# BBCG/epialleleR

Measured on AMD Instinct MI355X. Metric: Mreads/s generateCytosineReport (150 bp PE), higher is better.
Workload: dtype u8

## Files before the change

### epialleler_amd/csrc/cx_report.hip

```cpp
#include "common.hpp"
#include "tile_common.hpp"
#include <stdio.h>
#include <stdlib.h>
#include <string.h>

namespace epi {

#ifndef EPI_CX_WG
#define EPI_CX_WG 512
#endif
#ifndef EPI_CX_T1
#define EPI_CX_T1 2048
#endif
constexpr int CX_WG = EPI_CX_WG;
constexpr int CX_T1 = EPI_CX_T1;
constexpr int CX_CH = 16;
constexpr int CX_FLUSH_ROWS = 255;
constexpr int CX_SLAB_COV = 12;

struct __attribute__((packed, aligned(1))) U4u { uint32_t x, y, z, w; };

#ifndef EPI_CX_ABLATE
#define EPI_CX_ABLATE 0
#endif

struct Cx2Args {
  RowCols c;
  int64_t xm_cap;
  const Tile *tiles;
  uint32_t fill4;
  ClassLut lut_r;
  ClassLut lut_rx, lut_sx;
  ClassLut lut_s;
  ThrParams thr;
  const uint32_t *thr_tab;
  uint32_t ctx_of_plane;
  int32_t *pass_out;
  uint32_t *pool_key, *pool_meth, *pool_unmeth;
  uint32_t pool_cap;
  uint32_t *cursor;
  uint32_t slot_rows, ovf_base;
  uint32_t *tile_nrow, *tile_base;
  int32_t *slab;
  int heavy_rows;
  int heavy_chunk;
  int heavy_first;
  uint32_t *heavy_count, *heavy_max;
  uint32_t *heavy_list;
  int32_t *heavy_slab;
  uint32_t *deep_count, *deep_list;
  const uint32_t *tile_list, *tile_list_count;
  uint32_t *dbg;
  int64_t nrows;
  const uint32_t *prev_off, *prev_nrow;
  uint32_t *mismatch;
  int32_t *out[6];
  int64_t out_cap;
};

template <int T, int NP, bool LEAN = false> struct Cx2Lds {
  static constexpr int Q = T / 4;
  static constexpr int N_NARROW = 2 * NP * Q;
  static constexpr int N_CORR = 2 * Q;
  static constexpr int N_WIDE = LEAN ? 16 : 2 * NP * T;
  static constexpr int N_COV = T;
  unsigned long long *narrow, *corr;
  uint32_t *wide, *cov;
  uint32_t tid;
};

__device__ __forceinline__ uint32_t cx2_lut(uint32_t w, const ClassLut &X, uint32_t low8) {
  const uint32_t sel = (w & 0x0F0F0F0Fu) | low8;
  return __builtin_amdgcn_perm(X.lo1, X.lo0, sel) ^ __builtin_amdgcn_perm(X.hi1, X.hi0, sel ^ 0x08080808u);
}

template <int G>
__device__ __forceinline__ uint32_t cx2_group_sum(uint32_t v) {
  v += (uint32_t)__builtin_amdgcn_update_dpp(0, (int)v, 0xB1, 0xF, 0xF, true);
  v += (uint32_t)__builtin_amdgcn_update_dpp(0, (int)v, 0x4E, 0xF, 0xF, true);
  if (G >= 8) v += (uint32_t)__builtin_amdgcn_update_dpp(0, (int)v, 0x141, 0xF, 0xF, true);
  if (G >= 16) v += (uint32_t)__builtin_amdgcn_update_dpp(0, (int)v, 0x140, 0xF, 0xF, true);
  if (G >= 32) v += __shfl_xor(v, 16, 64);
  if (G >= 64) v += __shfl_xor(v, 32, 64);
  return v;
}

__device__ __forceinline__ int cx2_threshold(uint32_t n_m, uint32_t n_u, uint32_t o_m, uint32_t o_u, const ThrParams &prm) {
  int res = 0;
  if (n_m != 0) {
    const unsigned n_all = n_m + n_u;
    if (!(n_all < prm.min_n_ctx)) {
      const double frac = (double)n_m / (double)n_all;
      if (!(frac < prm.min_ctx_meth_frac)) {
        res = 1;
        if (o_m > 0) {
          const unsigned o_all = o_m + o_u;
          const double ofrac = (double)o_m / (double)o_all;
          if (ofrac > prm.max_ooctx_meth_frac) res = 0;
        }
      }
    }
  }
  return res;
}

__device__ __forceinline__ int cx2_threshold_tab(uint32_t n_m, uint32_t n_u, uint32_t o_m, uint32_t o_u, const ThrParams &prm,
                                                 const uint32_t *__restrict__ tab) {
  const uint32_t n_all = n_m + n_u, o_all = o_m + o_u;
  const uint32_t least = tab[n_all] & 0xFFFFu, most = tab[o_all] >> 16;
  return n_m != 0u && !(n_all < prm.min_n_ctx) && n_m >= least && (o_m == 0u || o_m <= most);
}

__global__ __launch_bounds__(256) void k_thr_table(ThrParams prm, int32_t nmax, uint32_t *__restrict__ tab) {
  const int32_t n = (int32_t)(blockIdx.x * 256 + threadIdx.x);
  if (n > nmax) return;
  uint32_t least = 0xFFFFu, most = 0u;
  if (n >= 1) {
    int32_t lo = 1, hi = n + 1;
    while (lo < hi) {
      const int32_t m = (lo + hi) >> 1;
// ... 117 lines not shown
#pragma unroll
    for (int u = 0; u < NU; u++) {
#pragma unroll
      for (int d = 0; d < 4; d++) w[u][d] = (EPI_CX_ABLATE & 4) ? w[u][d] : cx2_lut(w[u][d], a.lut_sx, 0u);
      fl |= w[u][0] | w[u][1] | w[u][2] | w[u][3];
    }
    auto count = [&](auto masked) {
      constexpr bool MASKED = decltype(masked)::value;
      constexpr uint32_t EV = MASKED ? 0x55555555u : 0xFFFFFFFFu;
      uint32_t E = 0, O = 0;
#pragma unroll
      for (int u = 0; u < NU; u++) {
        const uint32_t t = (w[u][0] & EV) + (w[u][1] & EV) + (w[u][2] & EV);
        const uint32_t d3 = w[u][3] & EV;
        E += (t & 0x33333333u) + (d3 & 0x33333333u);
        O += ((t >> 2) & 0x33333333u) + ((d3 >> 2) & 0x33333333u);
        if (u % 3 == 2 || u == NU - 1) {
          cls[0] = __builtin_amdgcn_sad_u8(E & 0x0F0F0F0Fu, 0u, cls[0]);
          cls[2] = __builtin_amdgcn_sad_u8((E >> 4) & 0x0F0F0F0Fu, 0u, cls[2]);
          cls[1] = __builtin_amdgcn_sad_u8(O & 0x0F0F0F0Fu, 0u, cls[1]);
          cls[3] = __builtin_amdgcn_sad_u8((O >> 4) & 0x0F0F0F0Fu, 0u, cls[3]);
          E = 0; O = 0;
        }
      }
    };
    if constexpr (MODE != 2) {
      if (__builtin_expect(__ballot((fl & 0xAAAAAAAAu) != 0u) == 0ull, 1)) count(std::false_type{});
      else count(std::true_type{});
    }
    if constexpr (MODE == 1) {
#pragma unroll
      for (int k = 0; k < 4; k++) carry[k] += cls[k];
      return;
    }
    if constexpr (MODE == 0) {
      const uint32_t s01 = cx2_group_sum<G>(cls[0] | (cls[1] << 16)), s23 = cx2_group_sum<G>(cls[2] | (cls[3] << 16));
      const uint32_t n_all = s01 & 0xFFFFu, n_m = s01 >> 16;
      g.ps = a.thr_tab ? cx2_threshold_tab(n_m, n_all - n_m, s23 & 0xFFFFu, s23 >> 16, a.thr, a.thr_tab)
                       : cx2_threshold(n_m, n_all - n_m, s23 & 0xFFFFu, s23 >> 16, a.thr);
      if (a.pass_out && sub == 0 && (uint32_t)g.rel < (uint32_t)T) a.pass_out[rcur] = g.ps;
    }
    const uint32_t pm = g.ps ? 0x01010101u : 0u;
#pragma unroll
    for (int u = 0; u < NU; u++) {
      const bool inside = (uint32_t)(cb + u * G) < (uint32_t)C;
#pragma unroll
      for (int d = 0; d < 4; d++) {
        const uint32_t lo = w[u][d] & 0x01010101u, hi = (w[u][d] >> 2) & pm;
        if (lo != 0u && inside && !(EPI_CX_ABLATE & 2)) atomicAdd(nar + 4 * u * G + d, (unsigned long long)lo | ((unsigned long long)hi << 32));
      }
    }
    const uint32_t fsel = g.ps ? 0x0A0A0A0Au : 0xA0A0A0A0u;
    if (__builtin_expect((fl & fsel) != 0u, 0)) {
      const int sh = g.ps ? 1 : 5;
#pragma unroll
      for (int u = 0; u < NU; u++) {
        const bool inside = (uint32_t)(cb + u * G) < (uint32_t)C;
#pragma unroll
        for (int d = 0; d < 4; d++) {
          const uint32_t sk = (w[u][d] >> sh) & 0x01010101u, db = (w[u][d] >> (sh + 2)) & 0x01010101u;
          if ((sk | db) != 0u && inside) atomicAdd(cor + 4 * u * G + d, (unsigned long long)sk | ((unsigned long long)db << 32));
        }
      }
    }
  } else if constexpr (NP == 1 && G >= 16) {
    const bool passing = g.ps != 0;
    const uint32_t k77 = (a.ctx_of_plane & 255u) * 0x11111111u;
    const uint32_t rm = passing ? 0xDDDDDDDDu : 0x55555555u, rv = passing ? 0x99999999u : 0x11111111u;
    uint32_t clean = 0xFFFFFFFFu;
#pragma unroll
    for (int u = 0; u < NU; u++) {
      const bool inside = (uint32_t)(cb + u * G) < (uint32_t)C;
#pragma unroll
      for (int e = 0; e < 2; e++) {
        const uint32_t pk = (w[u][2 * e] & 0x0F0F0F0Fu) | ((w[u][2 * e + 1] << 4) & 0xF0F0F0F0u);
        const uint32_t z = ((pk & 0x77777777u) ^ k77) + 0x77777777u;
        const uint32_t np = ~z & 0x88888888u;
        const uint32_t t = (pk & rm) ^ rv;
        clean &= ((t & 0x77777777u) + 0x77777777u) | t;
        if (np != 0u && inside && !(EPI_CX_ABLATE & 2)) {
          const uint32_t up = passing ? np & ~pk : 0u;
          const uint32_t n0 = (np >> 3) & 0x01010101u, n1 = (np >> 7) & 0x01010101u;
          if (n0 != 0u) atomicAdd(nar + 4 * u * G + 2 * e, (unsigned long long)n0 | ((unsigned long long)((up >> 3) & 0x01010101u) << 32));
          if (n1 != 0u) atomicAdd(nar + 4 * u * G + 2 * e + 1, (unsigned long long)n1 | ((unsigned long long)((up >> 7) & 0x01010101u) << 32));
        }
      }
    }
    if (__builtin_expect((~clean & 0x88888888u) != 0u, 0)) {
      const uint32_t pick0 = passing ? 0u : 0x08080808u;
#pragma unroll
      for (int u = 0; u < NU; u++) {
        const bool inside = (uint32_t)(cb + u * G) < (uint32_t)C;
#pragma unroll
        for (int d = 0; d < 4; d++) {
          const uint32_t f = cx2_lut(w[u][d], a.lut_rx, pick0);
          const uint32_t sk = (f >> 6) & 0x01010101u, db = (f >> 7) & 0x01010101u;
          if ((sk | db) != 0u && inside) atomicAdd(cor + 4 * u * G + d, (unsigned long long)sk | ((unsigned long long)db << 32));
        }
      }
    }
  } else {
    const uint32_t pick0 = g.ps == 0 ? 0x08080808u : 0u;
    uint32_t fl = 0;
#pragma unroll
    for (int u = 0; u < NU; u++) {
      const bool inside = (uint32_t)(cb + u * G) < (uint32_t)C;
#pragma unroll
      for (int d = 0; d < 4; d++) {
        const uint32_t f = cx2_lut(w[u][d], a.lut_rx, pick0);
        w[u][d] = f;
        fl |= f;
#pragma unroll
        for (int p = 0; p < NP; p++) {
          const uint32_t lo = (f >> (2 * p)) & 0x01010101u, hi = (f >> (2 * p + 1)) & 0x01010101u;
          if (lo != 0u && inside && !(EPI_CX_ABLATE & 2))
            atomicAdd(nar + p * Q + 4 * u * G + d, (unsigned long long)lo | ((unsigned long long)hi << 32));
        }
      }
    }
    if (__builtin_expect((fl & 0xC0C0C0C0u) != 0u, 0)) {
#pragma unroll
      for (int u = 0; u < NU; u++) {
        const bool inside = (uint32_t)(cb + u * G) < (uint32_t)C;
#pragma unroll
        for (int d = 0; d < 4; d++) {
          const uint32_t sk = (w[u][d] >> 6) & 0x01010101u, db = (w[u][d] >> 7) & 0x01010101u;
          if ((sk | db) != 0u && inside) atomicAdd(cor + 4 * u * G + d, (unsigned long long)sk | ((unsigned long long)db << 32));
        }
      }
    }
  }
}

template <int T, int G, int NU, int NP, bool FUSED, int WG, class LT>
__device__ __forceinline__ void cx2_rows(const Cx2Args &a, const Tile &td, int row_lo, int row_hi, const LT &L) {
  constexpr int R = 64 / G, NW = WG / 64, C = T / CX_CH;
  const int lane = L.tid & 63, wave = L.tid >> 6;
  const int sub = lane & (G - 1), grp = lane / G;
  Tile tb = td;
  tb.row_hi = row_hi;
  int r = row_lo + wave * R + grp;
  RowVals v = cx_load_row(a.c, tb, r);
  for (int rbase = row_lo + wave * R; rbase < row_hi; rbase += NW * R) {
    const int rcur = r;
    if (!EPI_DEV_CHECK(a.dbg, !v.ok || (rcur >= 0 && rcur < a.nrows && v.len >= 0 && (v.sd == 1 || v.sd == 2 || v.len == 0)), 22, rcur, v.sd)) return;
    r += NW * R;
    RowVals nv;
    bool fetched = false;
    auto fetch_next = [&]() { if (!fetched) { nv = cx_load_row(a.c, tb, r); fetched = true; } };
    if (v.ok && v.len > 0 && (int32_t)((uint32_t)v.st - (uint32_t)td.pos0) + v.len > 0) {
      Cx2Row g;
      g.rel = (int32_t)((uint32_t)v.st - (uint32_t)td.pos0);
      g.len = v.len;
      g.c0 = g.rel >> 4;
      g.clast = (g.rel + v.len - 1) >> 4;
      g.base = a.c.xm + (v.o - g.rel);
      g.edge = v.o < CX_CH || v.o + v.len + CX_CH > a.xm_cap;
      g.sidx = v.sd - 1;
      g.ps = v.ps;
      if constexpr (FUSED) {
        if (__builtin_expect(__ballot(g.clast - g.c0 >= G * NU) == 0ull, 1)) {
          cx2_visit<T, G, NU, NP, true>(a, g, g.c0, g.clast, sub, rcur, L, fetch_next);
        } else {
          uint32_t cls[4] = {0, 0, 0, 0};
          for (int32_t cs = g.c0; __ballot(cs <= g.clast) != 0ull; cs += G * NU)
            cx2_visit<T, G, NU, NP, true, 1>(a, g, cs, g.clast, sub, rcur, L, fetch_next, cls);
          const uint32_t s01 = cx2_group_sum<G>(cls[0] | (cls[1] << 16)), s23 = cx2_group_sum<G>(cls[2] | (cls[3] << 16));
          const uint32_t n_all = s01 & 0xFFFFu, n_m = s01 >> 16;
          g.ps = a.thr_tab ? cx2_threshold_tab(n_m, n_all - n_m, s23 & 0xFFFFu, s23 >> 16, a.thr, a.thr_tab)
                           : cx2_threshold(n_m, n_all - n_m, s23 & 0xFFFFu, s23 >> 16, a.thr);
          if (a.pass_out && sub == 0 && (uint32_t)g.rel < (uint32_t)T) a.pass_out[rcur] = g.ps;
          const int32_t ca = g.c0 > 0 ? g.c0 : 0, cz = g.clast < C - 1 ? g.clast : C - 1;
          for (int32_t cs = ca; __ballot(cs <= cz) != 0ull; cs += G * NU)
// ... 7 lines not shown
          for (int32_t cs = ca; __ballot(cs <= cz) != 0ull; cs += G * NU) cx2_visit<T, G, NU, NP, false>(a, g, cs, cz, sub, rcur, L, fetch_next);
        }
      }
      if (sub == 0) {
        const int32_t ca = g.rel > 0 ? g.rel : 0, cb = g.rel + v.len < T ? g.rel + v.len : T;
        const uint32_t unit = g.sidx ? 65536u : 1u;
        if (ca < cb && !(EPI_CX_ABLATE & 32)) { atomicAdd(L.cov + ca, unit); if (cb < T) atomicAdd(L.cov + cb, 0u - unit); }
      }
    } else if (FUSED && v.ok && sub == 0 && a.pass_out && (uint32_t)((uint32_t)v.st - (uint32_t)td.pos0) < (uint32_t)T) {
      a.pass_out[rcur] = 0;
    }
    fetch_next();
    v = nv;
  }
}

template <int T, int NP, bool LEAN, int WG>
__device__ __forceinline__ void cx2_flush(const Cx2Lds<T, NP, LEAN> &L) {
  constexpr int Q = Cx2Lds<T, NP, LEAN>::Q;
  if constexpr (!LEAN) {
    for (int i = L.tid; i < 2 * NP * Q; i += WG) {
      const unsigned long long v = L.narrow[i];
      if (v == 0ull) continue;
      L.narrow[i] = 0ull;
      const uint32_t lo = (uint32_t)v, hi = (uint32_t)(v >> 32);
      const int sp = i / Q, q = i - sp * Q;
      uint4 *wd = reinterpret_cast<uint4 *>(L.wide + sp * T + 4 * q);
      uint4 c = *wd;
      c.x += (lo & 255u) | ((hi & 255u) << 16);
      c.y += ((lo >> 8) & 255u) | (((hi >> 8) & 255u) << 16);
      c.z += ((lo >> 16) & 255u) | (((hi >> 16) & 255u) << 16);
      c.w += (lo >> 24) | ((hi >> 24) << 16);
      *wd = c;
    }
  }
  for (int i = L.tid; i < 2 * Q; i += WG) {
    const unsigned long long v = L.corr[i];
    if (v == 0ull) continue;
    L.corr[i] = 0ull;
    const uint32_t sk = (uint32_t)v, db = (uint32_t)(v >> 32);
    const int s = i / Q, q = i - s * Q;
    const int32_t unit = s ? 65536 : 1;
    int32_t prev = 0;
#pragma unroll
    for (int j = 0; j < 4; j++) {
      const int32_t d = (int32_t)((db >> (8 * j)) & 255u) - (int32_t)((sk >> (8 * j)) & 255u);
      if (d != prev) atomicAdd(L.cov + 4 * q + j, (uint32_t)((d - prev) * unit));
      prev = d;
    }
    if (prev != 0 && 4 * q + 4 < T) atomicAdd(L.cov + 4 * q + 4, (uint32_t)(-prev * unit));
  }
}

__device__ __forceinline__ uint32_t cx_pool_reserve(const Cx2Args &a, int tile, uint32_t n, bool *fits) {
  if (n <= a.slot_rows) { *fits = true; return (uint32_t)tile * a.slot_rows; }
  const uint32_t o = atomicAdd(a.cursor, n);
  *fits = (uint64_t)a.ovf_base + o + n <= a.pool_cap;
  return a.ovf_base + o;
}

__device__ __forceinline__ void cx_direct_none(const Cx2Args &a, int tile, uint32_t tid = threadIdx.x) {
  if (a.prev_off && tid == 0 && a.prev_nrow[tile] != 0u) atomicAdd(a.mismatch, 1u);
}

template <int T, int NP> struct CxSrcLds {
  const uint32_t *wide, *cov;
  __device__ __forceinline__ uint32_t any(int sd, int pos) const {
    uint32_t x = 0;
#pragma unroll
    for (int p = 0; p < NP; p++) x |= wide[(sd * NP + p) * T + pos];
    return x;
  }
  __device__ __forceinline__ void pair(int sd, int p, int pos, uint32_t *n, uint32_t *M) const {
    const uint32_t w = wide[(sd * NP + p) * T + pos];
    *n = w & 0xFFFFu; *M = w >> 16;
  }
  __device__ __forceinline__ uint32_t coverage(int sd, int pos) const { const uint32_t v = cov[pos]; return sd ? v >> 16 : v & 0xFFFFu; }
};
template <int QS> struct CxSrcU8 {
  const uint32_t *narrow;
  const uint32_t *cov;
  __device__ __forceinline__ uint32_t any(int sd, int pos) const {
    return (narrow[2 * (sd * QS + (pos >> 2))] >> (8 * (pos & 3))) & 255u;
  }
  __device__ __forceinline__ void pair(int sd, int, int pos, uint32_t *n, uint32_t *M) const {
    const uint2 c = *reinterpret_cast<const uint2 *>(narrow + 2 * (sd * QS + (pos >> 2)));
    *n = (c.x >> (8 * (pos & 3))) & 255u; *M = (c.y >> (8 * (pos & 3))) & 255u;
  }
  __device__ __forceinline__ uint32_t coverage(int sd, int pos) const { const uint32_t v = cov[pos]; return sd ? v >> 16 : v & 0xFFFFu; }
};
template <int T, int NP> struct CxSrcSlab {
  const int32_t *slab;
  const uint32_t *cov;
  __device__ __forceinline__ uint32_t any(int sd, int pos) const {
    uint32_t x = 0;
#pragma unroll
    for (int p = 0; p < NP; p++) x |= (uint32_t)slab[(2 * (sd * NP + p)) * T + pos];
    return x;
  }
  __device__ __forceinline__ void pair(int sd, int p, int pos, uint32_t *n, uint32_t *M) const {
    *n = (uint32_t)slab[(2 * (sd * NP + p)) * T + pos]; *M = (uint32_t)slab[(2 * (sd * NP + p) + 1) * T + pos];
  }
  __device__ __forceinline__ uint32_t coverage(int sd, int pos) const { return cov[sd * T + pos]; }
};

template <int T, int WG = CX_WG>
__device__ __forceinline__ void cx2_prefix(uint32_t *arr, uint32_t *s_scan, uint32_t tid = threadIdx.x) {
  constexpr int PPT = T / WG, NW = WG / 64;
  static_assert(PPT >= 1 && PPT <= 8, "prefix layout");
  const int lane = tid & 63, wave = tid >> 6;
  uint32_t x[PPT];
#pragma unroll
  for (int j = 0; j < PPT; j++) x[j] = arr[tid * PPT + j];
#pragma unroll
  for (int j = 1; j < PPT; j++) x[j] += x[j - 1];
  const uint32_t inc = wave_scan_u32(x[PPT - 1]);
  if (lane == 63) s_scan[wave] = inc;
  __syncthreads();
  uint32_t before = inc - x[PPT - 1];
#pragma unroll
  for (int w = 0; w < NW; w++) before += w < wave ? s_scan[w] : 0u;
#pragma unroll
  for (int j = 0; j < PPT; j++) arr[tid * PPT + j] = x[j] + before;
  __syncthreads();
}

template <int T, int NP, int WG = CX_WG, class SRC>
__device__ __forceinline__ void cx2_emit(const Cx2Args &a, int tile, const SRC &src, uint32_t *s_scan, uint16_t *s_list, uint32_t tid = threadIdx.x) {
  constexpr int NW = WG / 64, PW = T / NW, IT = PW / 32;
  static_assert(PW % 32 == 0 && IT >= 1 && IT <= 16, "emit phase layout");
  const int lane = tid & 63, wave = tid >> 6;
  const int l5 = lane & 31, sd = lane >> 5;
  const uint32_t below = (1u << l5) - 1u;
  uint16_t *list = s_list + wave * (2 * PW);
  uint32_t nc = 0;
#pragma unroll
  for (int i = 0; i < IT; i++) {
    const uint32_t any = src.any(sd, wave * PW + i * 32 + l5);
    const unsigned long long bal = __ballot(any != 0u);
    const uint32_t blo = (uint32_t)bal, bhi = (uint32_t)(bal >> 32);
    const uint32_t rank = (uint32_t)__popc(blo & below) + (uint32_t)__popc(bhi & below) + (sd ? (blo >> l5) & 1u : 0u);
    if (any != 0u) list[nc + rank] = (uint16_t)(i * 64 + lane);
    nc += (uint32_t)__popcll(bal);
  }
  uint32_t key[IT], me[IT], un[IT], off[IT];
  bool ok[IT];
  uint32_t carry = 0;
#pragma unroll
  for (int jj = 0; jj < IT; jj++) {
    ok[jj] = false; key[jj] = 0; me[jj] = 0; un[jj] = 0; off[jj] = 0;
    if ((uint32_t)(jj * 64) < nc) {
      const uint32_t j = (uint32_t)(jj * 64 + lane);
      bool good = false;
      if (j < nc) {
        const uint32_t id = list[j];
        const int pos = wave * PW + (int)(id >> 6) * 32 + (int)(id & 31u), st = (int)((id >> 5) & 1u);
        const uint32_t half = src.coverage(st, pos) >> 1;
        uint32_t ctx = 0, m = 0, u = 0;
#pragma unroll
        for (int p = 0; p < NP; p++) {
          uint32_t nn, M;
          src.pair(st, p, pos, &nn, &M);
          if (nn > half && ctx == 0) { ctx = (a.ctx_of_plane >> (8 * p)) & 255u; m = M; u = nn - M; }
        }
        good = ctx != 0;
        key[jj] = ((uint32_t)pos << 4) | ((uint32_t)st << 3) | ctx;
        me[jj] = m;
        un[jj] = u;
      }
      const unsigned long long be = __ballot(good);
      off[jj] = carry + __builtin_amdgcn_mbcnt_hi((uint32_t)(be >> 32), __builtin_amdgcn_mbcnt_lo((uint32_t)be, 0u));
      carry += (uint32_t)__popcll(be);
      ok[jj] = good;
    }
  }
  if (lane == 0) s_scan[wave] = carry;
  __syncthreads();
  if (a.prev_off) {
    if (tid == 0) {
      uint32_t acc = 0;
      for (int w = 0; w < NW; w++) { const uint32_t t = s_scan[w]; s_scan[w] = acc; acc += t; }
      const uint32_t base = a.prev_off[tile];
      const bool good = acc == a.prev_nrow[tile] && (int64_t)base + acc <= a.out_cap;
      if (!good) atomicAdd(a.mismatch, 1u);
      s_scan[NW + 1] = good ? base : 0xFFFFFFFFu;
    }
    __syncthreads();
    const uint32_t base = s_scan[NW + 1];
    if (base != 0xFFFFFFFFu) {
      const Tile td = a.tiles[tile];
      const uint32_t w0 = base + s_scan[wave];
#pragma unroll
      for (int jj = 0; jj < IT; jj++) {
        if (ok[jj]) {
          const uint32_t o = w0 + off[jj];
          a.out[0][o] = td.rname;
          a.out[1][o] = 1 + (int32_t)((key[jj] >> 3) & 1u);
          a.out[2][o] = (int32_t)(td.pos0 + (int64_t)(key[jj] >> 4));
          a.out[3][o] = (int32_t)(key[jj] & 7u);
          a.out[4][o] = (int32_t)me[jj];
          a.out[5][o] = (int32_t)un[jj];
        }
      }
    }
    return;
  }
  if (tid == 0) {
    uint32_t acc = 0;
    for (int w = 0; w < NW; w++) { const uint32_t t = s_scan[w]; s_scan[w] = acc; acc += t; }
    s_scan[NW] = acc;
    uint32_t base = 0;
    bool fits = true;
    if (acc) base = cx_pool_reserve(a, tile, acc, &fits);
    s_scan[NW + 1] = base;
    s_scan[NW] = fits ? acc : 0xFFFFFFFFu;
    a.tile_nrow[tile] = acc;
    a.tile_base[tile] = base;
  }
  __syncthreads();
  const uint32_t total = s_scan[NW], base = s_scan[NW + 1];
  if (total != 0xFFFFFFFFu) {
    const uint32_t w0 = base + s_scan[wave];
#pragma unroll
    for (int jj = 0; jj < IT; jj++) {
      if (ok[jj]) {
        const uint32_t w = w0 + off[jj];
        if (!EPI_DEV_CHECK(a.dbg, w < a.pool_cap, 23, w, a.pool_cap)) continue;
        a.pool_key[w] = key[jj];
        a.pool_meth[w] = me[jj];
        a.pool_unmeth[w] = un[jj];
      }
    }
  }
}

template <int T, int NP, bool LEAN, int WG>
__device__ __forceinline__ void cx2_dump_slab(const Cx2Lds<T, NP, LEAN> &L, int32_t *slab) {
  uint32_t *dst = reinterpret_cast<uint32_t *>(slab);
  if constexpr (LEAN) {
    constexpr int Q = Cx2Lds<T, NP, LEAN>::Q;
    for (int i = L.tid; i < 2 * NP * Q; i += WG) {
      const unsigned long long v = L.narrow[i];
      if (v == 0ull) continue;
      const uint32_t lo = (uint32_t)v, hi = (uint32_t)(v >> 32);
      const int sp = i / Q, q = i - sp * Q;
#pragma unroll
      for (int j = 0; j < 4; j++) {
        const uint32_t n = (lo >> (8 * j)) & 255u, M = (hi >> (8 * j)) & 255u;
        if (n) atomicAdd(dst + (2 * sp) * T + 4 * q + j, n);
        if (M) atomicAdd(dst + (2 * sp + 1) * T + 4 * q + j, M);
      }
    }
  } else {
    for (int i = L.tid; i < 2 * NP * T; i += WG) {
      const uint32_t v = L.wide[i];
      if (!v) continue;
      const int sp = i / T, p = i - sp * T;
      if (v & 0xFFFFu) atomicAdd(dst + (2 * sp) * T + p, v & 0xFFFFu);
      if (v >> 16) atomicAdd(dst + (2 * sp + 1) * T + p, v >> 16);
    }
  }
  for (int p = L.tid; p < T; p += WG) {
    const uint32_t v = L.cov[p];
    if (!v) continue;
    const int32_t lo = (int32_t)(int16_t)(v & 0xFFFFu);
    const int32_t hi = ((int32_t)v - lo) >> 16;
    if (lo) atomicAdd(dst + CX_SLAB_COV * T + p, (uint32_t)lo);
    if (hi) atomicAdd(dst + (CX_SLAB_COV + 1) * T + p, (uint32_t)hi);
  }
}

__device__ __forceinline__ int cx_tile_of_block(int b, int ntiles) {
  const int chunk = (ntiles + 7) >> 3;
  return (b & 7) * chunk + (b >> 3);
}

template <int T, int NP, bool LEAN = false> constexpr int cx2_lds_bytes() {
  using LdsT = Cx2Lds<T, NP, LEAN>;
  return (LdsT::N_NARROW + LdsT::N_CORR) * 8 + (LdsT::N_WIDE + LdsT::N_COV) * 4;
}
#ifndef EPI_CX_WPS
#define EPI_CX_WPS 8
#endif
template <int T, int NP, int NU = 3, bool LEAN = false, int WG = CX_WG> constexpr int cx2_waves_per_simd() {
  const int by_lds = (160 * 1024) / (cx2_lds_bytes<T, NP, LEAN>() + 64), by_thr = 2048 / WG;
  int wgs = by_lds < by_thr ? by_lds : by_thr;
  if (NU >= 4 && wgs * WG > 1536) wgs = 1536 / WG;
  if (wgs * WG / 256 > EPI_CX_WPS) wgs = EPI_CX_WPS * 256 / WG;
  return (wgs < 1 ? 1 : wgs) * WG / 256;
}

#define CX2_SHARED(T, NP, LEAN)                                                                                  \
  using LdsT = Cx2Lds<T, NP, LEAN>;                                                                              \
  __shared__ __attribute__((aligned(16))) unsigned long long s_u8[LdsT::N_NARROW + LdsT::N_CORR];                \
  __shared__ __attribute__((aligned(16))) uint32_t s_wide[LdsT::N_WIDE];                                         \
  __shared__ __attribute__((aligned(16))) uint32_t s_cov[LdsT::N_COV];                                           \
  static_assert((LdsT::N_NARROW + LdsT::N_CORR) * 8 >= 4 * T + 64 && LdsT::N_CORR * 8 >= 4 * T, "the candidate lists and the scan scratch reuse dead arrays"); \
  uint32_t *s_scan = LEAN ? s_wide : reinterpret_cast<uint32_t *>(s_u8) + T;                                      \
  uint16_t *s_list = reinterpret_cast<uint16_t *>(LEAN ? s_u8 + LdsT::N_NARROW : s_u8);                          \
  (void)s_scan; (void)s_list;                                                                                     \
  LdsT L;                                                                                                         \
  L.narrow = s_u8; L.corr = s_u8 + LdsT::N_NARROW; L.wide = s_wide; L.cov = s_cov; L.tid = threadIdx.x;

template <int T, int NP, bool LEAN, int WG>
__device__ __forceinline__ void cx2_clear(const Cx2Lds<T, NP, LEAN> &L) {
  using LdsT = Cx2Lds<T, NP, LEAN>;
  uint4 *z = reinterpret_cast<uint4 *>(L.narrow);
  for (int i = L.tid; i < (LdsT::N_NARROW + LdsT::N_CORR) / 2; i += WG) z[i] = make_uint4(0, 0, 0, 0);
  if constexpr (!LEAN) {
    uint4 *y = reinterpret_cast<uint4 *>(L.wide);
    for (int i = L.tid; i < LdsT::N_WIDE / 4; i += WG) y[i] = make_uint4(0, 0, 0, 0);
  }
  uint4 *x = reinterpret_cast<uint4 *>(L.cov);
  for (int i = L.tid; i < LdsT::N_COV / 4; i += WG) x[i] = make_uint4(0, 0, 0, 0);
}

template <int T, int G, int NU, int NP, bool FUSED, bool LEAN, int WG>
__device__ __forceinline__ void cx2_accumulate(const Cx2Args &a, const Tile &td, int row_lo, int row_hi, const Cx2Lds<T, NP, LEAN> &L) {
  if constexpr (LEAN) {
    cx2_rows<T, G, NU, NP, FUSED, WG>(a, td, row_lo, row_hi, L);
  } else {
    for (int b0 = row_lo; b0 < row_hi; b0 += CX_FLUSH_ROWS) {
      if (b0 > row_lo) { __syncthreads(); cx2_flush<T, NP, LEAN, WG>(L); __syncthreads(); }
      cx2_rows<T, G, NU, NP, FUSED, WG>(a, td, b0, b0 + CX_FLUSH_ROWS < row_hi ? b0 + CX_FLUSH_ROWS : row_hi, L);
    }
  }
  __syncthreads();
  cx2_flush<T, NP, LEAN, WG>(L);
  __syncthreads();
}

#ifndef EPI_CX_LEAN_WG
#define EPI_CX_LEAN_WG 256
#endif
template <bool LEAN> constexpr int cx2_wg() { return LEAN ? EPI_CX_LEAN_WG : CX_WG; }

template <int T, int G, int NU, int NP, bool FUSED, bool LEAN, class LdsT>
__device__ __forceinline__ void cx2_tile(const Cx2Args &a, int tile, const Tile &td, const LdsT &L, uint32_t *s_scan, uint16_t *s_list, int *s_flag) {
  constexpr int WG = cx2_wg<LEAN>();
  cx2_clear<T, NP, LEAN, WG>(L);
  if (td.row_hi - td.row_lo > a.heavy_rows) {
    if (L.tid == 0) {
      const uint32_t h = atomicAdd(a.heavy_count, 1u);
      a.heavy_list[h] = (uint32_t)tile;
      atomicMax(a.heavy_max, (uint32_t)(td.row_hi - td.row_lo));
      a.tile_nrow[tile] = 0;
      a.tile_base[tile] = 0;
    }
    cx_direct_none(a, tile, L.tid);
    return;
  }
  if constexpr (LEAN) {
    if (a.deep_list && td.row_hi - td.row_lo > CX_FLUSH_ROWS) {
      if (L.tid == 0) *s_flag = 0;
      __syncthreads();
      bool deep = false;
      for (int x = td.row_lo + (int)L.tid; x + CX_FLUSH_ROWS < td.row_hi; x += WG)
        deep |= (int64_t)a.c.start[x + CX_FLUSH_ROWS] < (int64_t)a.c.start[x] + a.c.len[x];
      if (deep) *s_flag = 1;
      __syncthreads();
      if (*s_flag) {
        if (L.tid == 0) { a.deep_list[atomicAdd(a.deep_count, 1u)] = (uint32_t)tile; a.tile_nrow[tile] = 0; a.tile_base[tile] = 0; }
        cx_direct_none(a, tile, L.tid);
        return;
      }
    }
  }
  __syncthreads();
  cx2_accumulate<T, G, NU, NP, FUSED, LEAN, WG>(a, td, td.row_lo, td.row_hi, L);
  if (td.slot >= 0) {
    cx2_dump_slab<T, NP, LEAN, WG>(L, a.slab + (int64_t)td.slot * (kCxPlanes * T));
    if (L.tid == 0) { a.tile_nrow[tile] = 0; a.tile_base[tile] = 0; }
    cx_direct_none(a, tile, L.tid);
    return;
  }
  if (EPI_CX_ABLATE & 16) { if (L.tid == 0) { a.tile_nrow[tile] = 0; a.tile_base[tile] = 0; } cx_direct_none(a, tile, L.tid); return; }
  cx2_prefix<T, WG>(L.cov, s_scan, L.tid);
  if constexpr (LEAN) {
    static_assert(NP == 1, "the u8 counters serve single-context reports");
    CxSrcU8<LdsT::Q> src;
    src.narrow = reinterpret_cast<const uint32_t *>(L.narrow); src.cov = L.cov;
    cx2_emit<T, NP, WG>(a, tile, src, s_scan, s_list, L.tid);
  } else {
    CxSrcLds<T, NP> src;
    src.wide = L.wide; src.cov = L.cov;
    cx2_emit<T, NP, WG>(a, tile, src, s_scan, s_list, L.tid);
  }
}

template <int T, int G, int NU, int NP, bool FUSED, bool LEAN>
__global__ __launch_bounds__(cx2_wg<LEAN>(), (cx2_waves_per_simd<T, NP, NU, LEAN, cx2_wg<LEAN>()>())) void k_cx_tiles(Cx2Args a, int ntiles) {
  CX2_SHARED(T, NP, LEAN)
  __shared__ int s_flag;
  if constexpr (!LEAN) {
    if (a.tile_list) {
      const uint32_t n = *a.tile_list_count;
      for (uint32_t i = blockIdx.x; i < n; i += gridDim.x) {
        const int tile = (int)a.tile_list[i];
        const Tile td = a.tiles[tile];
        cx2_tile<T, G, NU, NP, FUSED, LEAN>(a, tile, td, L, s_scan, s_list, &s_flag);
        __syncthreads();
      }
      return;
    }
  }
  const int tile = cx_tile_of_block(blockIdx.x, ntiles);
  if (tile >= ntiles) return;
  const Tile td = a.tiles[tile];
  cx2_tile<T, G, NU, NP, FUSED, LEAN>(a, tile, td, L, s_scan, s_list, &s_flag);
}

template <int T, int G, int NU, int NP, bool FUSED>
__global__ __launch_bounds__(CX_WG, (cx2_waves_per_simd<T, NP, NU>())) void k_cx_heavy(Cx2Args a) {
  CX2_SHARED(T, NP, false)
  const uint32_t hi_idx = (uint32_t)a.heavy_first + blockIdx.y;
  if (hi_idx >= *a.heavy_count) return;
  const int tile = (int)a.heavy_list[hi_idx];
  const Tile td = a.tiles[tile];
  for (int lo = td.row_lo + (int)blockIdx.x * a.heavy_chunk; lo < td.row_hi; lo += (int)gridDim.x * a.heavy_chunk) {
    const int hi = td.row_hi - lo > a.heavy_chunk ? lo + a.heavy_chunk : td.row_hi;
    cx2_clear<T, NP, false, CX_WG>(L);
    __syncthreads();
    cx2_accumulate<T, G, NU, NP, FUSED, false, CX_WG>(a, td, lo, hi, L);
    cx2_dump_slab<T, NP, false, CX_WG>(L, td.slot >= 0 ? a.slab + (int64_t)td.slot * (kCxPlanes * T)
                                          : a.heavy_slab + (int64_t)blockIdx.y * (kCxPlanes * T));
    __syncthreads();
  }
}

template <int T, int NP>
__device__ __forceinline__ void cx2_emit_from_slab(const Cx2Args &a, int tile, const int32_t *slab) {
  __shared__ __attribute__((aligned(16))) uint32_t s_cov[2 * T];
  __shared__ uint32_t s_scan[CX_WG / 64 + 2];
  __shared__ uint16_t s_list[2 * T];
  for (int i = threadIdx.x; i < 2 * T; i += CX_WG) s_cov[i] = (uint32_t)slab[CX_SLAB_COV * T + i];
  __syncthreads();
  cx2_prefix<T>(s_cov, s_scan);
  cx2_prefix<T>(s_cov + T, s_scan);
  CxSrcSlab<T, NP> src;
  src.slab = slab; src.cov = s_cov;
  cx2_emit<T, NP>(a, tile, src, s_scan, s_list);
}

template <int T, int NP>
__global__ __launch_bounds__(CX_WG) void k_cx_emit_heavy(Cx2Args a) {
  const uint32_t hi_idx = (uint32_t)a.heavy_first + blockIdx.x;
  if (hi_idx >= *a.heavy_count) return;
  const int tile = (int)a.heavy_list[hi_idx];
  if (a.tiles[tile].slot >= 0) return;
  cx2_emit_from_slab<T, NP>(a, tile, a.heavy_slab + (int64_t)blockIdx.x * (kCxPlanes * T));
}

template <int T, int NP>
__global__ __launch_bounds__(CX_WG) void k_cx_emit_slab(Cx2Args a, const int32_t *__restrict__ owned,
                                                         const int32_t *__restrict__ slot_tile) {
  if (!owned[blockIdx.x]) return;
  const int tile = slot_tile[blockIdx.x];
  if (tile < 0) return;
  cx2_emit_from_slab<T, NP>(a, tile, a.slab + (int64_t)a.tiles[tile].slot * (kCxPlanes * T));
}

#ifndef EPI_CXP_T
#define EPI_CXP_T 1024
#endif
constexpr int CXP_T = EPI_CXP_T;

template <int G, int U0, int U1>
__device__ __forceinline__ void cxp_add_range(const uint32_t (&w)[CX_NU], const RowSlice &cur) {
  if constexpr (U0 < U1) {
    if (U0 * G <= cur.tl) cx_add_dword<CXP_T, 4 * G * U0, U0 == 0>(w[U0], cur.tl == U0 * G, cur);
    cxp_add_range<G, U0 + 1, U1>(w, cur);
  }
}

template <int G>
__device__ __forceinline__ void cxp_accumulate(const RowCols &c, const Tile &td, uint32_t *cnt) {
  constexpr int R = 64 / G, NW = CX_WG / 64;
  const int lane = threadIdx.x & 63, wave = threadIdx.x >> 6;
  const int sub = lane & (G - 1), grp = lane / G;
  int r = td.row_lo + wave * R + grp;
  RowSlice cur = cx_row_slice<CXP_T, G>(c, td, r, sub, cnt);
  for (int rbase = td.row_lo + wave * R; rbase < td.row_hi; rbase += NW * R) {
    uint32_t w[CX_NU];
#pragma unroll
    for (int u = 0; u < CX_NU; u++) w[u] = u * G <= cur.tl ? cur.src[u * G] : 0u;
    r += NW * R;
    const RowSlice nxt = cx_row_slice<CXP_T, G>(c, td, r, sub, cnt);
    cxp_add_range<G, 0, CX_NU>(w, cur);
    for (int k = sub + CX_NU * G; k < cur.nd; k += G) {
      RowSlice t = cur;
#pragma unroll
      for (int j = 0; j < 4; j++) t.dst[j] = cur.dst[j] + 4 * (k - sub);
      cx_add_dword<CXP_T, 0, false>(cur.src[k - sub], k == cur.nd - 1, t);
    }
// ... 18 lines not shown
  const uint32_t *cnt;
  int pl[3];
  __device__ __forceinline__ uint32_t any(int sd, int pos) const {
    uint32_t x = 0;
#pragma unroll
    for (int p = 0; p < 3; p++) if (pl[p]) x |= cnt[(sd * 4 + pl[p]) * CXP_T + pos];
    return x;
  }
  __device__ __forceinline__ void pair(int sd, int p, int pos, uint32_t *n, uint32_t *M) const {
    const uint32_t w = pl[p] ? cnt[(sd * 4 + pl[p]) * CXP_T + pos] : 0u;
    *n = w & 0xFFFFu; *M = w >> 16;
  }
  __device__ __forceinline__ uint32_t coverage(int sd, int pos) const { return cnt[sd * 4 * CXP_T + pos]; }
};

__device__ __forceinline__ CxSrcPk cxp_source(const Cx2Args &a, const uint32_t *cnt) {
  CxSrcPk s;
  s.cnt = cnt;
#pragma unroll
  for (int p = 0; p < 3; p++) { const uint32_t k = (a.ctx_of_plane >> (8 * p)) & 255u; s.pl[p] = k == 2u ? 1 : k == 6u ? 2 : k == 7u ? 3 : 0; }
  return s;
}

__device__ __forceinline__ void cxp_dump_slab(const Cx2Args &a, const uint32_t *cnt, int np, int32_t *slab) {
  constexpr int T = CXP_T;
  uint32_t *dst = reinterpret_cast<uint32_t *>(slab);
  const CxSrcPk src = cxp_source(a, cnt);
  for (int i = threadIdx.x; i < 2 * T; i += CX_WG) {
    const int sd = i / T, pos = i % T;
#pragma unroll
    for (int p = 0; p < 3; p++) {
      if (p >= np) break;
      uint32_t n, M;
      src.pair(sd, p, pos, &n, &M);
      if (n) atomicAdd(dst + (2 * (sd * np + p)) * T + pos, n);
      if (M) atomicAdd(dst + (2 * (sd * np + p) + 1) * T + pos, M);
    }
    const uint32_t d = src.coverage(sd, pos) - (pos ? src.coverage(sd, pos - 1) : 0u);
    if (d) atomicAdd(dst + (CX_SLAB_COV + sd) * T + pos, d);
  }
}

#define CXP_SHARED                                                                                      \
  __shared__ __attribute__((aligned(16))) uint32_t cnt_raw[8 * CXP_T + 2 * kCxGuard];                  \
  __shared__ uint32_t s_scan[CX_WG / 64 + 2];                                                         \
  __shared__ uint16_t s_list[2 * CXP_T];                                                               \
  uint32_t *cnt = cnt_raw + kCxGuard;

template <int G>
__global__ __launch_bounds__(CX_WG, 8) void k_cxp_tiles(Cx2Args a, int ntiles, int np) {
  CXP_SHARED
  const int tile = cx_tile_of_block(blockIdx.x, ntiles);
  if (tile >= ntiles) return;
  const Tile td = a.tiles[tile];
  uint4 *z = reinterpret_cast<uint4 *>(cnt_raw);
  for (int i = threadIdx.x; i < (8 * CXP_T + 2 * kCxGuard) / 4; i += CX_WG) z[i] = make_uint4(0, 0, 0, 0);
  if (td.row_hi - td.row_lo > a.heavy_rows) {
    if (threadIdx.x == 0) {
      const uint32_t h = atomicAdd(a.heavy_count, 1u);
      a.heavy_list[h] = (uint32_t)tile;
      atomicMax(a.heavy_max, (uint32_t)(td.row_hi - td.row_lo));
      a.tile_nrow[tile] = 0;
      a.tile_base[tile] = 0;
    }
    cx_direct_none(a, tile);
    return;
  }
  __syncthreads();
  cxp_accumulate<G>(a.c, td, cnt);
  __syncthreads();
  cxp_convert(cnt);
  __syncthreads();
  if (td.slot >= 0) {
    cxp_dump_slab(a, cnt, np, a.slab + (int64_t)td.slot * (kCxPlanes * CXP_T));
    if (threadIdx.x == 0) { a.tile_nrow[tile] = 0; a.tile_base[tile] = 0; }
    cx_direct_none(a, tile);
    return;
  }
  if (EPI_CX_ABLATE & 16) {
    if (threadIdx.x == 0) { a.tile_nrow[tile] = 0; a.tile_base[tile] = 0; }
    cx_direct_none(a, tile);
    return;
  }
  cx2_emit<CXP_T, 3>(a, tile, cxp_source(a, cnt), s_scan, s_list);
}

template <int G>
__global__ __launch_bounds__(CX_WG, 8) void k_cxp_heavy(Cx2Args a, int np) {
  CXP_SHARED
  (void)s_scan; (void)s_list;
  const uint32_t hi_idx = (uint32_t)a.heavy_first + blockIdx.y;
  if (hi_idx >= *a.heavy_count) return;
  const int tile = (int)a.heavy_list[hi_idx];
  const Tile whole = a.tiles[tile];
  for (int lo = whole.row_lo + (int)blockIdx.x * a.heavy_chunk; lo < whole.row_hi; lo += (int)gridDim.x * a.heavy_chunk) {
    Tile td = whole;
    td.row_lo = lo;
    if (td.row_hi - lo > a.heavy_chunk) td.row_hi = lo + a.heavy_chunk;
    uint4 *z = reinterpret_cast<uint4 *>(cnt_raw);
    for (int i = threadIdx.x; i < (8 * CXP_T + 2 * kCxGuard) / 4; i += CX_WG) z[i] = make_uint4(0, 0, 0, 0);
    __syncthreads();
    cxp_accumulate<G>(a.c, td, cnt);
    __syncthreads();
    cxp_convert(cnt);
    __syncthreads();
    cxp_dump_slab(a, cnt, np, td.slot >= 0 ? a.slab + (int64_t)td.slot * (kCxPlanes * CXP_T)
                                            : a.heavy_slab + (int64_t)blockIdx.y * (kCxPlanes * CXP_T));
    __syncthreads();
  }
}

struct __attribute__((packed, aligned(4))) CxU4u { uint32_t x, y, z, w; };

__global__ __launch_bounds__(256) void k_cx_gather(const Tile *__restrict__ tiles, const uint32_t *__restrict__ tile_out,
                                                    const uint32_t *__restrict__ tile_nrow, const uint32_t *__restrict__ tile_base,
                                                    int32_t ntiles, const uint32_t *__restrict__ pool_key,
                                                    const uint32_t *__restrict__ pool_meth, const uint32_t *__restrict__ pool_unmeth,
                                                    int32_t *__restrict__ o_rname, int32_t *__restrict__ o_strand,
                                                    int32_t *__restrict__ o_pos, int32_t *__restrict__ o_ctx,
                                                    int32_t *__restrict__ o_meth, int32_t *__restrict__ o_unmeth) {
  const int tile = blockIdx.x * 4 + (threadIdx.x >> 6);
  if (tile >= ntiles) return;
  const uint32_t n = tile_nrow[tile];
  if (n == 0) return;
  const int lane = threadIdx.x & 63;
  const Tile td = tiles[tile];
  const uint32_t src0 = tile_base[tile], dst0 = tile_out[tile];
  const uint32_t n4 = n & ~3u;
  for (uint32_t i = 4u * lane; i < n4; i += 256) {
    const CxU4u key = *reinterpret_cast<const CxU4u *>(pool_key + src0 + i);
    const CxU4u me = *reinterpret_cast<const CxU4u *>(pool_meth + src0 + i);
    const CxU4u un = *reinterpret_cast<const CxU4u *>(pool_unmeth + src0 + i);
    const uint32_t o = dst0 + i;
    const uint32_t rn = (uint32_t)td.rname;
    const uint32_t p0 = (uint32_t)td.pos0;
    *reinterpret_cast<CxU4u *>(o_rname + o) = CxU4u{rn, rn, rn, rn};
    *reinterpret_cast<CxU4u *>(o_strand + o) = CxU4u{1u + ((key.x >> 3) & 1u), 1u + ((key.y >> 3) & 1u), 1u + ((key.z >> 3) & 1u), 1u + ((key.w >> 3) & 1u)};
// ... 692 lines not shown
```

Before: 12410.

## Trim barriers and serial scan in cytosine emit; park tile metadata in LDS

```diff
diff --git a/epialleler_amd/csrc/cx_report.hip b/epialleler_amd/csrc/cx_report.hip
--- a/epialleler_amd/csrc/cx_report.hip
+++ b/epialleler_amd/csrc/cx_report.hip
@@ -64,8 +64,10 @@
   static constexpr int N_CORR = 2 * Q;
   static constexpr int N_WIDE = LEAN ? 16 : 2 * NP * T;
   static constexpr int N_COV = T;
+  static constexpr bool kLean = LEAN;
   unsigned long long *narrow, *corr;
   uint32_t *wide, *cov;
+  uint32_t *corr_used;
   uint32_t tid;
 };
 
@@ -289,6 +291,7 @@
     }
     const uint32_t fsel = g.ps ? 0x0A0A0A0Au : 0xA0A0A0A0u;
     if (__builtin_expect((fl & fsel) != 0u, 0)) {
+      if constexpr (LT::kLean) *L.corr_used = 1u;
       const int sh = g.ps ? 1 : 5;
 #pragma unroll
       for (int u = 0; u < NU; u++) {
@@ -324,6 +327,7 @@
       }
     }
     if (__builtin_expect((~clean & 0x88888888u) != 0u, 0)) {
+      if constexpr (LT::kLean) *L.corr_used = 1u;
       const uint32_t pick0 = passing ? 0u : 0x08080808u;
 #pragma unroll
       for (int u = 0; u < NU; u++) {
@@ -356,6 +360,7 @@
       }
     }
     if (__builtin_expect((fl & 0xC0C0C0C0u) != 0u, 0)) {
+      if constexpr (LT::kLean) *L.corr_used = 1u;
 #pragma unroll
       for (int u = 0; u < NU; u++) {
         const bool inside = (uint32_t)(cb + u * G) < (uint32_t)C;
@@ -469,15 +474,26 @@
   }
 }
 
-__device__ __forceinline__ uint32_t cx_pool_reserve(const Cx2Args &a, int tile, uint32_t n, bool *fits) {
-  if (n <= a.slot_rows) { *fits = true; return (uint32_t)tile * a.slot_rows; }
+__device__ __forceinline__ uint32_t cx_pool_overflow(const Cx2Args &a, uint32_t n, bool *fits) {
   const uint32_t o = atomicAdd(a.cursor, n);
   *fits = (uint64_t)a.ovf_base + o + n <= a.pool_cap;
   return a.ovf_base + o;
 }
 
-__device__ __forceinline__ void cx_direct_none(const Cx2Args &a, int tile, uint32_t tid = threadIdx.x) {
-  if (a.prev_off && tid == 0 && a.prev_nrow[tile] != 0u) atomicAdd(a.mismatch, 1u);
+constexpr int CX_PARK_WORDS = 8;
+enum { CX_PK_RNAME = 0, CX_PK_POS_LO, CX_PK_POS_HI, CX_PK_OFF, CX_PK_NROW };
+__device__ __forceinline__ void cx_park(const Cx2Args &a, int tile, const Tile &td, uint32_t *park, uint32_t tid = threadIdx.x) {
+  if (tid == 0) {
+    park[CX_PK_RNAME] = (uint32_t)td.rname;
+    park[CX_PK_POS_LO] = (uint32_t)td.pos0;
+    park[CX_PK_POS_HI] = (uint32_t)((uint64_t)td.pos0 >> 32);
+    if (a.prev_off) { park[CX_PK_OFF] = a.prev_off[tile]; park[CX_PK_NROW] = a.prev_nrow[tile]; }
+  }
+}
+
+template <bool PARKED>
+__device__ __forceinline__ void cx_direct_none(const Cx2Args &a, int tile, const uint32_t *park, uint32_t tid = threadIdx.x) {
+  if (a.prev_off && tid == 0 && (PARKED ? park[CX_PK_NROW] : a.prev_nrow[tile]) != 0u) atomicAdd(a.mismatch, 1u);
 }
 
 template <int T, int NP> struct CxSrcLds {
@@ -521,7 +537,7 @@
   __device__ __forceinline__ uint32_t coverage(int sd, int pos) const { return cov[sd * T + pos]; }
 };
 
-template <int T, int WG = CX_WG>
+template <int T, int WG = CX_WG, bool OWN_RANGE = false>
 __device__ __forceinline__ void cx2_prefix(uint32_t *arr, uint32_t *s_scan, uint32_t tid = threadIdx.x) {
   constexpr int PPT = T / WG, NW = WG / 64;
   static_assert(PPT >= 1 && PPT <= 8, "prefix layout");
@@ -539,11 +555,19 @@
   for (int w = 0; w < NW; w++) before += w < wave ? s_scan[w] : 0u;
 #pragma unroll
   for (int j = 0; j < PPT; j++) arr[tid * PPT + j] = x[j] + before;
-  __syncthreads();
-}
-
-template <int T, int NP, int WG = CX_WG, class SRC>
-__device__ __forceinline__ void cx2_emit(const Cx2Args &a, int tile, const SRC &src, uint32_t *s_scan, uint16_t *s_list, uint32_t tid = threadIdx.x) {
+  if constexpr (OWN_RANGE) {
+    static_assert(64 * PPT == T / NW, "a wavefront prefixes exactly the range the emit's wavefront reads");
+    __builtin_amdgcn_fence(__ATOMIC_RELEASE, "wavefront");
+    __builtin_amdgcn_wave_barrier();
+    __builtin_amdgcn_fence(__ATOMIC_ACQUIRE, "wavefront");
+  } else {
+    __syncthreads();
+  }
+}
+
+template <int T, int NP, int WG = CX_WG, bool PARKED = false, class SRC>
+__device__ __forceinline__ void cx2_emit(const Cx2Args &a, int tile, const SRC &src, uint32_t *s_scan, uint16_t *s_list, const uint32_t *park,
+                                         uint32_t tid = threadIdx.x) {
   constexpr int NW = WG / 64, PW = T / NW, IT = PW / 32;
   static_assert(PW % 32 == 0 && IT >= 1 && IT <= 16, "emit phase layout");
   const int lane = tid & 63, wave = tid >> 6;
@@ -593,51 +617,55 @@
   }
   if (lane == 0) s_scan[wave] = carry;
   __syncthreads();
+  uint32_t acc = 0, mine = 0;
+#pragma unroll
+  for (int w = 0; w < NW; w++) { const uint32_t t = s_scan[w]; mine += w < wave ? t : 0u; acc += t; }
+  acc = __builtin_amdgcn_readfirstlane(acc);
+  mine = __builtin_amdgcn_readfirstlane(mine);
   if (a.prev_off) {
+    uint32_t base, want, rname, plo, phi;
+    if constexpr (PARKED) {
+      base = park[CX_PK_OFF]; want = park[CX_PK_NROW];
+      rname = park[CX_PK_RNAME]; plo = park[CX_PK_POS_LO]; phi = park[CX_PK_POS_HI];
+    } else {
+      const Tile td = a.tiles[tile];
+      base = a.prev_off[tile]; want = a.prev_nrow[tile];
+      rname = (uint32_t)td.rname; plo = (uint32_t)td.pos0; phi = (uint32_t)((uint64_t)td.pos0 >> 32);
+    }
+    if (!(acc == want && (int64_t)base + acc <= a.out_cap)) {
+      if (tid == 0) atomicAdd(a.mismatch, 1u);
+      return;
+    }
+    const int64_t pos0 = (int64_t)(((uint64_t)phi << 32) | plo);
+    const uint32_t w0 = base + mine;
+#pragma unroll
+    for (int jj = 0; jj < IT; jj++) {
+      if (ok[jj]) {
+        const uint32_t o = w0 + off[jj];
+        a.out[0][o] = (int32_t)rname;
+        a.out[1][o] = 1 + (int32_t)((key[jj] >> 3) & 1u);
+        a.out[2][o] = (int32_t)(pos0 + (int64_t)(key[jj] >> 4));
+        a.out[3][o] = (int32_t)(key[jj] & 7u);
+        a.out[4][o] = (int32_t)me[jj];
+        a.out[5][o] = (int32_t)un[jj];
+      }
+    }
+    return;
+  }
+  uint32_t base = acc ? (uint32_t)tile * a.slot_rows : 0u;
+  bool fits = true;
+  if (acc > a.slot_rows) {
     if (tid == 0) {
-      uint32_t acc = 0;
-      for (int w = 0; w < NW; w++) { const uint32_t t = s_scan[w]; s_scan[w] = acc; acc += t; }
-      const uint32_t base = a.prev_off[tile];
-      const bool good = acc == a.prev_nrow[tile] && (int64_t)base + acc <= a.out_cap;
-      if (!good) atomicAdd(a.mismatch, 1u);
-      s_scan[NW + 1] = good ? base : 0xFFFFFFFFu;
+      s_scan[NW] = cx_pool_overflow(a, acc, &fits);
+      s_scan[NW + 1] = fits ? 1u : 0u;
     }
     __syncthreads();
-    const uint32_t base = s_scan[NW + 1];
-    if (base != 0xFFFFFFFFu) {
-      const Tile td = a.tiles[tile];
-      const uint32_t w0 = base + s_scan[wave];
-#pragma unroll
-      for (int jj = 0; jj < IT; jj++) {
-        if (ok[jj]) {
-          const uint32_t o = w0 + off[jj];
-          a.out[0][o] = td.rname;
-          a.out[1][o] = 1 + (int32_t)((key[jj] >> 3) & 1u);
-          a.out[2][o] = (int32_t)(td.pos0 + (int64_t)(key[jj] >> 4));
-          a.out[3][o] = (int32_t)(key[jj] & 7u);
-          a.out[4][o] = (int32_t)me[jj];
-          a.out[5][o] = (int32_t)un[jj];
-        }
-      }
-    }
-    return;
-  }
-  if (tid == 0) {
-    uint32_t acc = 0;
-    for (int w = 0; w < NW; w++) { const uint32_t t = s_scan[w]; s_scan[w] = acc; acc += t; }
-    s_scan[NW] = acc;
-    uint32_t base = 0;
-    bool fits = true;
-    if (acc) base = cx_pool_reserve(a, tile, acc, &fits);
-    s_scan[NW + 1] = base;
-    s_scan[NW] = fits ? acc : 0xFFFFFFFFu;
-    a.tile_nrow[tile] = acc;
-    a.tile_base[tile] = base;
-  }
-  __syncthreads();
-  const uint32_t total = s_scan[NW], base = s_scan[NW + 1];
-  if (total != 0xFFFFFFFFu) {
-    const uint32_t w0 = base + s_scan[wave];
+    base = s_scan[NW];
+    fits = s_scan[NW + 1] != 0u;
+  }
+  if (tid == 0) { a.tile_nrow[tile] = acc; a.tile_base[tile] = base; }
+  if (fits) {
+    const uint32_t w0 = base + mine;
 #pragma unroll
     for (int jj = 0; jj < IT; jj++) {
       if (ok[jj]) {
@@ -712,12 +740,13 @@
   __shared__ __attribute__((aligned(16))) unsigned long long s_u8[LdsT::N_NARROW + LdsT::N_CORR];                \
   __shared__ __attribute__((aligned(16))) uint32_t s_wide[LdsT::N_WIDE];                                         \
   __shared__ __attribute__((aligned(16))) uint32_t s_cov[LdsT::N_COV];                                           \
-  static_assert((LdsT::N_NARROW + LdsT::N_CORR) * 8 >= 4 * T + 64 && LdsT::N_CORR * 8 >= 4 * T, "the candidate lists and the scan scratch reuse dead arrays"); \
+  __shared__ uint32_t s_corr_used;                                                                                \
+  static_assert((LdsT::N_NARROW + LdsT::N_CORR) * 8 >= 4 * T + 128 && LdsT::N_CORR * 8 >= 4 * T, "the candidate lists and the scan scratch reuse dead arrays"); \
   uint32_t *s_scan = LEAN ? s_wide : reinterpret_cast<uint32_t *>(s_u8) + T;                                      \
   uint16_t *s_list = reinterpret_cast<uint16_t *>(LEAN ? s_u8 + LdsT::N_NARROW : s_u8);                          \
   (void)s_scan; (void)s_list;                                                                                     \
   LdsT L;                                                                                                         \
-  L.narrow = s_u8; L.corr = s_u8 + LdsT::N_NARROW; L.wide = s_wide; L.cov = s_cov; L.tid = threadIdx.x;
+  L.narrow = s_u8; L.corr = s_u8 + LdsT::N_NARROW; L.wide = s_wide; L.cov = s_cov; L.corr_used = &s_corr_used; L.tid = threadIdx.x;
 
 template <int T, int NP, bool LEAN, int WG>
 __device__ __forceinline__ void cx2_clear(const Cx2Lds<T, NP, LEAN> &L) {
@@ -730,12 +759,18 @@
   }
   uint4 *x = reinterpret_cast<uint4 *>(L.cov);
   for (int i = L.tid; i < LdsT::N_COV / 4; i += WG) x[i] = make_uint4(0, 0, 0, 0);
+  if (LEAN && L.tid == 0) *L.corr_used = 0u;
 }
 
 template <int T, int G, int NU, int NP, bool FUSED, bool LEAN, int WG>
 __device__ __forceinline__ void cx2_accumulate(const Cx2Args &a, const Tile &td, int row_lo, int row_hi, const Cx2Lds<T, NP, LEAN> &L) {
   if constexpr (LEAN) {
     cx2_rows<T, G, NU, NP, FUSED, WG>(a, td, row_lo, row_hi, L);
+    __syncthreads();
+    if (__builtin_amdgcn_readfirstlane(*L.corr_used) == 0u) return;
+    cx2_flush<T, NP, LEAN, WG>(L);
+    __syncthreads();
+    return;
   } else {
     for (int b0 = row_lo; b0 < row_hi; b0 += CX_FLUSH_ROWS) {
       if (b0 > row_lo) { __syncthreads(); cx2_flush<T, NP, LEAN, WG>(L); __syncthreads(); }
@@ -752,9 +787,10 @@
 #endif
 template <bool LEAN> constexpr int cx2_wg() { return LEAN ? EPI_CX_LEAN_WG : CX_WG; }
 
-template <int T, int G, int NU, int NP, bool FUSED, bool LEAN, class LdsT>
-__device__ __forceinline__ void cx2_tile(const Cx2Args &a, int tile, const Tile &td, const LdsT &L, uint32_t *s_scan, uint16_t *s_list, int *s_flag) {
-  constexpr int WG = cx2_wg<LEAN>();
+template <int T, int G, int NU, int NP, bool FUSED, bool LEAN, bool PARKED, class LdsT>
+__device__ __forceinline__ void cx2_tile(const Cx2Args &a, int tile, const Tile &td, const LdsT &L, uint32_t *s_scan, uint16_t *s_list, int *s_flag,
+                                         const uint32_t *park) {
+  constexpr int WG = cx2_wg<LEAN>(), NW = WG / 64;
   cx2_clear<T, NP, LEAN, WG>(L);
   if (td.row_hi - td.row_lo > a.heavy_rows) {
     if (L.tid == 0) {
@@ -764,7 +800,7 @@
       a.tile_nrow[tile] = 0;
       a.tile_base[tile] = 0;
     }
-    cx_direct_none(a, tile, L.tid);
+    cx_direct_none<PARKED>(a, tile, park, L.tid);
     return;
   }
   if constexpr (LEAN) {
@@ -778,7 +814,7 @@
       __syncthreads();
       if (*s_flag) {
         if (L.tid == 0) { a.deep_list[atomicAdd(a.deep_count, 1u)] = (uint32_t)tile; a.tile_nrow[tile] = 0; a.tile_base[tile] = 0; }
-        cx_direct_none(a, tile, L.tid);
+        cx_direct_none<PARKED>(a, tile, park, L.tid);
         return;
       }
     }
@@ -788,20 +824,23 @@
   if (td.slot >= 0) {
     cx2_dump_slab<T, NP, LEAN, WG>(L, a.slab + (int64_t)td.slot * (kCxPlanes * T));
     if (L.tid == 0) { a.tile_nrow[tile] = 0; a.tile_base[tile] = 0; }
-    cx_direct_none(a, tile, L.tid);
+    cx_direct_none<PARKED>(a, tile, park, L.tid);
     return;
   }
-  if (EPI_CX_ABLATE & 16) { if (L.tid == 0) { a.tile_nrow[tile] = 0; a.tile_base[tile] = 0; } cx_direct_none(a, tile, L.tid); return; }
-  cx2_prefix<T, WG>(L.cov, s_scan, L.tid);
+  if (EPI_CX_ABLATE & 16) { if (L.tid == 0) { a.tile_nrow[tile] = 0; a.tile_base[tile] = 0; } cx_direct_none<PARKED>(a, tile, park, L.tid); return; }
+  static_assert(!LEAN || 2 * NW + 2 <= LdsT::N_WIDE, "scan scratch of the lean kernel");
+  static_assert(4 * (2 * NW + 2) <= 128, "scan scratch behind the candidate lists (CX2_SHARED)");
+  cx2_prefix<T, WG, true>(L.cov, s_scan, L.tid);
+  s_scan += NW;
   if constexpr (LEAN) {
     static_assert(NP == 1, "the u8 counters serve single-context reports");
     CxSrcU8<LdsT::Q> src;
     src.narrow = reinterpret_cast<const uint32_t *>(L.narrow); src.cov = L.cov;
-    cx2_emit<T, NP, WG>(a, tile, src, s_scan, s_list, L.tid);
+    cx2_emit<T, NP, WG, PARKED>(a, tile, src, s_scan, s_list, park, L.tid);
   } else {
     CxSrcLds<T, NP> src;
     src.wide = L.wide; src.cov = L.cov;
-    cx2_emit<T, NP, WG>(a, tile, src, s_scan, s_list, L.tid);
+    cx2_emit<T, NP, WG, PARKED>(a, tile, src, s_scan, s_list, park, L.tid);
   }
 }
 
@@ -815,7 +854,7 @@
       for (uint32_t i = blockIdx.x; i < n; i += gridDim.x) {
         const int tile = (int)a.tile_list[i];
         const Tile td = a.tiles[tile];
-        cx2_tile<T, G, NU, NP, FUSED, LEAN>(a, tile, td, L, s_scan, s_list, &s_flag);
+        cx2_tile<T, G, NU, NP, FUSED, LEAN, false>(a, tile, td, L, s_scan, s_list, &s_flag, nullptr);
         __syncthreads();
       }
       return;
@@ -823,8 +862,10 @@
   }
   const int tile = cx_tile_of_block(blockIdx.x, ntiles);
   if (tile >= ntiles) return;
+  __shared__ uint32_t s_park[CX_PARK_WORDS];
   const Tile td = a.tiles[tile];
-  cx2_tile<T, G, NU, NP, FUSED, LEAN>(a, tile, td, L, s_scan, s_list, &s_flag);
+  cx_park(a, tile, td, s_park);
+  cx2_tile<T, G, NU, NP, FUSED, LEAN, true>(a, tile, td, L, s_scan, s_list, &s_flag, s_park);
 }
 
 template <int T, int G, int NU, int NP, bool FUSED>
@@ -856,7 +897,7 @@
   cx2_prefix<T>(s_cov + T, s_scan);
   CxSrcSlab<T, NP> src;
   src.slab = slab; src.cov = s_cov;
-  cx2_emit<T, NP>(a, tile, src, s_scan, s_list);
+  cx2_emit<T, NP>(a, tile, src, s_scan, s_list, nullptr);
 }
 
 template <int T, int NP>
@@ -981,7 +1022,9 @@
   CXP_SHARED
   const int tile = cx_tile_of_block(blockIdx.x, ntiles);
   if (tile >= ntiles) return;
+  __shared__ uint32_t s_park[CX_PARK_WORDS];
   const Tile td = a.tiles[tile];
+  cx_park(a, tile, td, s_park);
   uint4 *z = reinterpret_cast<uint4 *>(cnt_raw);
   for (int i = threadIdx.x; i < (8 * CXP_T + 2 * kCxGuard) / 4; i += CX_WG) z[i] = make_uint4(0, 0, 0, 0);
   if (td.row_hi - td.row_lo > a.heavy_rows) {
@@ -992,7 +1035,7 @@
       a.tile_nrow[tile] = 0;
       a.tile_base[tile] = 0;
     }
-    cx_direct_none(a, tile);
+    cx_direct_none<true>(a, tile, s_park);
     return;
   }
   __syncthreads();
@@ -1003,15 +1046,15 @@
   if (td.slot >= 0) {
     cxp_dump_slab(a, cnt, np, a.slab + (int64_t)td.slot * (kCxPlanes * CXP_T));
     if (threadIdx.x == 0) { a.tile_nrow[tile] = 0; a.tile_base[tile] = 0; }
-    cx_direct_none(a, tile);
+    cx_direct_none<true>(a, tile, s_park);
     return;
   }
   if (EPI_CX_ABLATE & 16) {
     if (threadIdx.x == 0) { a.tile_nrow[tile] = 0; a.tile_base[tile] = 0; }
-    cx_direct_none(a, tile);
+    cx_direct_none<true>(a, tile, s_park);
     return;
   }
-  cx2_emit<CXP_T, 3>(a, tile, cxp_source(a, cnt), s_scan, s_list);
+  cx2_emit<CXP_T, 3, CX_WG, true>(a, tile, cxp_source(a, cnt), s_scan, s_list, s_park);
 }
 
 template <int G>
```

Result: faster. 12570 (median of 6 runs) (+1.3%).
